# savelovme/adaptive-mcmc

Hardware: AMD Instinct MI355X
Metric: chain-steps/sec (whole node) + ESS/sec, 64-dim Gaussian (higher is better)
Workload: dtype f32; 1 GPU; ARWMH.sample, d=64 correlated Gaussian, 65536 chains, per-chain adaptation (BASELINE.json configs[1]); chains_per_gpu=65536, dim=64, parallelism=1 GPU

## Files before the change

adaptive-mcmc_amd/csrc/amh_step64.hip:

```cpp
#include "amh_asss.h"
#include "amh_device.h"
#include "amh_s64_sched.h"
#include "amh_step_stage.h"

namespace amh {

#ifdef AMH_STAMPS
constexpr int kS64StampWaves = 1 << 16;
constexpr int kS64StampSlots = 16;
constexpr int kS64SubPhases = 6;
__device__ unsigned long long g_s64_stamps[kS64StampWaves * kS64StampSlots];
hipError_t diag_s64_stamps_copy(void* host, size_t bytes) {
  return hipMemcpyFromSymbol(host, HIP_SYMBOL(g_s64_stamps), bytes, 0, hipMemcpyDeviceToHost);
}
#define AMH_S64_PHASE_INIT                                  \
  unsigned long long st_ph[4] = {0, 0, 0, 0}, st_pt = 0; \
  S64Sub st_sub = {{0, 0, 0, 0, 0, 0}, 0};
#define AMH_S64_PHASE_MARK st_pt = __builtin_amdgcn_s_memrealtime();
#define AMH_S64_PHASE(k)                                             \
  {                                                                  \
    const unsigned long long t_ = __builtin_amdgcn_s_memrealtime();  \
    st_ph[k] += t_ - st_pt;                                          \
    st_pt = t_;                                                      \
  }
struct S64Sub {
  unsigned long long ph[kS64SubPhases], pt;
};
#define AMH_S64_SUB_PARAM , S64Sub& st_sub
#define AMH_S64_SUB_ARG , st_sub
#define AMH_S64_SUB_MARK st_sub.pt = __builtin_amdgcn_s_memrealtime();
#define AMH_S64_SUB(k)                                               \
  {                                                                  \
    const unsigned long long t_ = __builtin_amdgcn_s_memrealtime();  \
    st_sub.ph[k] += t_ - st_sub.pt;                                  \
    st_sub.pt = t_;                                                  \
  }
#else
#define AMH_S64_PHASE_INIT
#define AMH_S64_PHASE_MARK
#define AMH_S64_PHASE(k)
#define AMH_S64_SUB_PARAM
#define AMH_S64_SUB_ARG
#define AMH_S64_SUB_MARK
#define AMH_S64_SUB(k)
#endif

constexpr int kS64Waves = 16;
constexpr int kS64LoadAuxHot = 2, kS64LoadAuxCold = 2;
constexpr int kS64StoreAuxHot = 2, kS64StoreAuxMid = 0, kS64StoreAuxTail = 0;
constexpr int kS64TagShift = 60;
constexpr int64_t kS64IdxMask = ((int64_t)1 << kS64TagShift) - 1;
__device__ __forceinline__ int s64_cls(int64_t t) { return (int)(t >> kS64TagShift); }
template <class F>
__device__ __forceinline__ void s64_load_policy(int cls, F&& f) {
  using std::integral_constant;
  if constexpr (kS64LoadAuxHot == kS64LoadAuxCold) {
    f(integral_constant<int, kS64LoadAuxCold>{});
  } else {
    if (cls & (int)kS64Hot) f(integral_constant<int, kS64LoadAuxHot>{});
    else f(integral_constant<int, kS64LoadAuxCold>{});
  }
}
template <class F>
__device__ __forceinline__ void s64_store_policy(int cls, F&& f) {
  using std::integral_constant;
  if constexpr (kS64StoreAuxHot == kS64StoreAuxMid && kS64StoreAuxTail == kS64StoreAuxMid) {
    f(integral_constant<int, kS64StoreAuxMid>{});
  } else {
    if (cls & (int)kS64Hot) f(integral_constant<int, kS64StoreAuxHot>{});
    else if (cls & (int)kS64Tail) f(integral_constant<int, kS64StoreAuxTail>{});
    else f(integral_constant<int, kS64StoreAuxMid>{});
  }
}
constexpr int kS64EB = 8;
constexpr int kS64PB = 8;
constexpr int kS64PG = 16;
static_assert(kS64EB == 8 && kS64PB == 8, "the batch readers (lds_ld4x2w / lds_ld4x4w) read two quarter-vectors per stream");
static_assert(kS64PG == 16, "s64_gauss_pot_sg waits for four quarter-rows; s64_lanes takes 8 or 16");
typedef uint32_t uint32x4_t_ __attribute__((ext_vector_type(4)));
constexpr int kS64P = 2080;
constexpr int kS64Z = 2080, kS64M = 2144, kS64S = 2208, kS64X = 2216;
constexpr int kS64WB = kS64X + 64;
constexpr int kS64Model = 64 * 68;
static_assert(kS64Z == 2080 && kS64S == kS64M + 64, "layout of prefetch_item<64>");
template <int WPB = kS64Waves>
constexpr size_t s64_lds_bytes() { return ((size_t)kS64Model + (size_t)WPB * kS64WB + 32) * sizeof(float); }

constexpr int s64_col(int j) { return j * 64 - j * (j - 1) / 2; }

constexpr int kS64Pieces = 9;
constexpr int s64_piece_end(int m) { return m < kS64Pieces - 1 ? 256 * (m + 1) : kS64P; }
constexpr int s64_piece_group(int m) {
  for (int g = 0; g < 16; ++g)
    if (s64_col(4 * g + 4) >= s64_piece_end(m)) return g;
  return -1;
}
constexpr int s64_piece_after(int g) {
  for (int m = 0; m < kS64Pieces; ++m)
    if (s64_piece_group(m) == g) return m;
  return -1;
}
constexpr bool s64_pieces_ok() {
  int n = 0;
  for (int g = 0; g < 16; ++g) n += s64_piece_after(g) >= 0;
  for (int m = 0; m + 1 < kS64Pieces; ++m)
    if (s64_piece_group(m) < 0 || s64_piece_group(m) >= s64_piece_group(m + 1)) return false;
  return n == kS64Pieces;
}
static_assert(256 * (kS64Pieces - 1) <= kS64P && kS64P - 256 * (kS64Pieces - 1) <= 64, "eight 1-KB pieces and a one-DMA tail");
static_assert(s64_col(64) == kS64P && s64_pieces_ok(), "every piece is finished by its own swap group, in order");
static_assert(s64_piece_group(0) == 1 && s64_piece_group(4) == 6 && s64_piece_group(7) == 14 &&
                  s64_piece_group(kS64Pieces - 1) == 15,
              "the table of DESIGN.md 3.1");

#define AMH_SWG_RD(k) "ds_read_b32 %[t" #k "], %[la] offset:%[o" #k "]\n\t"
#define AMH_SWG_RD_HEAD "ds_read_b128 %[dl], %[zm] offset:%[od]\n\tds_read_b128 %[in], %[zm] offset:%[oi]\n\t"
#define AMH_SWG_RD_PIECE "ds_read_b128 %[pv], %[lp] offset:%[op]\n\t"
#define AMH_SWG_RD_TAIL "s_waitcnt lgkmcnt(0)"
template <int G, int MP>
__device__ __forceinline__ void s64_group_read(f32x4& dl4, f32x4& in4, f32x4& pv, float (&t)[4], uint32_t zm_a,
                                               uint32_t la16, uint32_t la) {
  constexpr int j = 4 * G;
  static_assert(G < 15 || MP >= 0, "the last group reads the piece that group 14 finished");
  static_assert(s64_col(j) >= j && s64_col(j + 3) - (j + 3) + 63 < kS64P, "unmasked column reads stay inside the factor");
#define AMH_SWG_RD_OPS3                                                                          \
  [zm] "v"(zm_a), [la] "v"(la), [od] "n"(16 * G), [oi] "n"(256 + 16 * G),                       \
      [o0] "n"((s64_col(j) - j) * 4), [o1] "n"((s64_col(j + 1) - (j + 1)) * 4),                 \
      [o2] "n"((s64_col(j + 2) - (j + 2)) * 4)
  if constexpr (G == 15) {
    asm volatile(AMH_SWG_RD_HEAD AMH_SWG_RD_PIECE AMH_SWG_RD(0) AMH_SWG_RD(1) AMH_SWG_RD(2) AMH_SWG_RD_TAIL
                 : [dl] "=&v"(dl4), [in] "=&v"(in4), [pv] "=&v"(pv), [t0] "=&v"(t[0]), [t1] "=&v"(t[1]),
                   [t2] "=&v"(t[2])
                 : AMH_SWG_RD_OPS3, [lp] "v"(la16), [op] "n"(1024 * MP));
  } else if constexpr (MP >= 0) {
    asm volatile(AMH_SWG_RD_HEAD AMH_SWG_RD_PIECE AMH_SWG_RD(0) AMH_SWG_RD(1) AMH_SWG_RD(2) AMH_SWG_RD(3)
                     AMH_SWG_RD_TAIL
                 : [dl] "=&v"(dl4), [in] "=&v"(in4), [pv] "=&v"(pv), [t0] "=&v"(t[0]), [t1] "=&v"(t[1]),
                   [t2] "=&v"(t[2]), [t3] "=&v"(t[3])
                 : AMH_SWG_RD_OPS3, [o3] "n"((s64_col(j + 3) - (j + 3)) * 4), [lp] "v"(la16), [op] "n"(1024 * MP));
  } else {
    asm volatile(AMH_SWG_RD_HEAD AMH_SWG_RD(0) AMH_SWG_RD(1) AMH_SWG_RD(2) AMH_SWG_RD(3) AMH_SWG_RD_TAIL
                 : [dl] "=&v"(dl4), [in] "=&v"(in4), [t0] "=&v"(t[0]), [t1] "=&v"(t[1]), [t2] "=&v"(t[2]),
                   [t3] "=&v"(t[3])
                 : AMH_SWG_RD_OPS3, [o3] "n"((s64_col(j + 3) - (j + 3)) * 4));
  }
#undef AMH_SWG_RD_OPS3
}
#define AMH_SWG_LP                                                                      \
  "v_mul_f32 %[d0], %[u0], %[d0]\n\tv_mul_f32 %[d1], %[u1], %[d1]\n\t"                  \
  "v_mul_f32 %[d2], %[u2], %[d2]\n\tv_mul_f32 %[d3], %[u3], %[d3]\n\t"
#define AMH_SWG_WR(k) "ds_write_b32 %[la], %[d" #k "] offset:%[o" #k "]\n\t"
#define AMH_SWG_NRM(k) "v_mul_f32 %[u" #k "], %[t" #k "], %[i" #k "]\n\t"
#define AMH_SWG_SH(k) "s_lshl_b64 exec, -1, %[m" #k "]\n\t"
#define AMH_SWG_OFFS                                                                                          \
  [o0] "n"((s64_col(j) - j) * 4), [o1] "n"((s64_col(j + 1) - (j + 1)) * 4),                                   \
      [o2] "n"((s64_col(j + 2) - (j + 2)) * 4), [o3] "n"((s64_col(j + 3) - (j + 3)) * 4), [m0] "n"(j),        \
      [m1] "n"(j + 1), [m2] "n"(j + 2), [m3] "n"(j + 3)
template <int G>
__device__ __forceinline__ void s64_group_write(const float (&U)[64], uint32_t la, const f32x4& dl4) {
  constexpr int j = 4 * G;
  float d0 = dl4[0], d1 = dl4[1], d2 = dl4[2], d3 = dl4[3];
  asm volatile(AMH_SWG_LP AMH_SWG_SH(0) AMH_SWG_WR(0) AMH_SWG_SH(1) AMH_SWG_WR(1) AMH_SWG_SH(2) AMH_SWG_WR(2)
                   AMH_SWG_SH(3) AMH_SWG_WR(3) "s_mov_b64 exec, -1"
               : [d0] "+v"(d0), [d1] "+v"(d1), [d2] "+v"(d2), [d3] "+v"(d3)
               : [la] "v"(la), [u0] "v"(U[j]), [u1] "v"(U[j + 1]), [u2] "v"(U[j + 2]), [u3] "v"(U[j + 3]), AMH_SWG_OFFS
               : "memory");
}
template <int G>
__device__ __forceinline__ void s64_group_norm(float (&U)[64], const f32x4& in4, const float (&t)[4]) {
  constexpr int j = 4 * G;
  if constexpr (G < 15) {
    asm volatile(AMH_SWG_SH(1) AMH_SWG_NRM(0) AMH_SWG_SH(2) AMH_SWG_NRM(1) AMH_SWG_SH(3) AMH_SWG_NRM(2) AMH_SWG_SH(4)
                     AMH_SWG_NRM(3) "s_mov_b64 exec, -1"
                 : [u0] "+v"(U[j]), [u1] "+v"(U[j + 1]), [u2] "+v"(U[j + 2]), [u3] "+v"(U[j + 3])
                 : [t0] "v"(t[0]), [t1] "v"(t[1]), [t2] "v"(t[2]), [t3] "v"(t[3]), [i0] "v"(in4[0]), [i1] "v"(in4[1]),
                   [i2] "v"(in4[2]), [i3] "v"(in4[3]), [m1] "n"(j + 1), [m2] "n"(j + 2), [m3] "n"(j + 3),
                   [m4] "n"(j + 4));
  } else {
    asm volatile(AMH_SWG_SH(1) AMH_SWG_NRM(0) AMH_SWG_SH(2) AMH_SWG_NRM(1) AMH_SWG_SH(3) AMH_SWG_NRM(2)
                 "s_mov_b64 exec, -1"
                 : [u0] "+v"(U[j]), [u1] "+v"(U[j + 1]), [u2] "+v"(U[j + 2])
                 : [t0] "v"(t[0]), [t1] "v"(t[1]), [t2] "v"(t[2]), [i0] "v"(in4[0]), [i1] "v"(in4[1]),
                   [i2] "v"(in4[2]), [m1] "n"(j + 1), [m2] "n"(j + 2), [m3] "n"(j + 3));
  }
}
template <int O0, int O1>
__device__ __forceinline__ void lds_ld4x2w(f32x4& a, f32x4& b, uint32_t addr) {
  asm volatile("ds_read_b128 %0, %2 offset:%3\n\tds_read_b128 %1, %2 offset:%4\n\ts_waitcnt lgkmcnt(0)"
               : "=&v"(a), "=&v"(b)
               : "v"(addr), "n"(O0), "n"(O1));
}
template <int O0, int O1, int O2, int O3>
__device__ __forceinline__ void lds_ld4x4w(f32x4& a, f32x4& b, f32x4& c, f32x4& d, uint32_t addr0, uint32_t addr1) {
  asm volatile("ds_read_b128 %0, %4 offset:%6\n\tds_read_b128 %1, %4 offset:%7\n\t"
               "ds_read_b128 %2, %5 offset:%8\n\tds_read_b128 %3, %5 offset:%9\n\ts_waitcnt lgkmcnt(0)"
               : "=&v"(a), "=&v"(b), "=&v"(c), "=&v"(d)
               : "v"(addr0), "v"(addr1), "n"(O0), "n"(O1), "n"(O2), "n"(O3));
}

#define AMH_SW1_COL(k)                                                          \
  "s_lshl_b64 exec, -1, %[s" #k "]\n\tv_readlane_b32 %[t], %[w], %[l" #k "]\n\t" \
  "s_nop 1\n\tv_fma_f32 %[w], -%[t], %[u" #k "], %[w]\n\ts_nop 0\n\t"
template <int J0>
__device__ __forceinline__ void s64_sweep1x8(float& w, const float (&U)[64]) {
  uint64_t sv;
  uint32_t t;
  if constexpr (J0 + 7 <= 62) {
    asm volatile("s_mov_b64 %[sv], exec\n\t" AMH_SW1_COL(0) AMH_SW1_COL(1) AMH_SW1_COL(2) AMH_SW1_COL(3)
                 AMH_SW1_COL(4) AMH_SW1_COL(5) AMH_SW1_COL(6) AMH_SW1_COL(7) "s_mov_b64 exec, %[sv]"
                 : [w] "+v"(w), [t] "=&s"(t), [sv] "=&s"(sv)
                 : [u0] "v"(U[J0]), [u1] "v"(U[J0 + 1]), [u2] "v"(U[J0 + 2]), [u3] "v"(U[J0 + 3]),
                   [u4] "v"(U[J0 + 4]), [u5] "v"(U[J0 + 5]), [u6] "v"(U[J0 + 6]), [u7] "v"(U[J0 + 7]),
                   [s0] "n"(J0 + 1), [s1] "n"(J0 + 2), [s2] "n"(J0 + 3), [s3] "n"(J0 + 4), [s4] "n"(J0 + 5),
                   [s5] "n"(J0 + 6), [s6] "n"(J0 + 7), [s7] "n"(J0 + 8), [l0] "n"(J0), [l1] "n"(J0 + 1),
                   [l2] "n"(J0 + 2), [l3] "n"(J0 + 3), [l4] "n"(J0 + 4), [l5] "n"(J0 + 5), [l6] "n"(J0 + 6),
                   [l7] "n"(J0 + 7));
  } else {
    static_assert(J0 == 56, "sweep 1 covers columns 0 .. 62");
    asm volatile("s_mov_b64 %[sv], exec\n\t" AMH_SW1_COL(0) AMH_SW1_COL(1) AMH_SW1_COL(2) AMH_SW1_COL(3)
                 AMH_SW1_COL(4) AMH_SW1_COL(5) AMH_SW1_COL(6) "s_mov_b64 exec, %[sv]"
                 : [w] "+v"(w), [t] "=&s"(t), [sv] "=&s"(sv)
                 : [u0] "v"(U[J0]), [u1] "v"(U[J0 + 1]), [u2] "v"(U[J0 + 2]), [u3] "v"(U[J0 + 3]),
                   [u4] "v"(U[J0 + 4]), [u5] "v"(U[J0 + 5]), [u6] "v"(U[J0 + 6]), [s0] "n"(J0 + 1),
                   [s1] "n"(J0 + 2), [s2] "n"(J0 + 3), [s3] "n"(J0 + 4), [s4] "n"(J0 + 5), [s5] "n"(J0 + 6),
                   [s6] "n"(J0 + 7), [l0] "n"(J0), [l1] "n"(J0 + 1), [l2] "n"(J0 + 2), [l3] "n"(J0 + 3),
                   [l4] "n"(J0 + 4), [l5] "n"(J0 + 5), [l6] "n"(J0 + 6));
  }
}
#undef AMH_SW1_COL
__device__ __forceinline__ void s64_sweep1_all(float& w, const float (&U)[64]) {
  static_for<8>([&](auto B) {
    s64_sweep1x8<8 * B>(w, U);
    __builtin_amdgcn_sched_barrier(0);
  });
}

template <int Q>
__device__ __forceinline__ void s64_wr4_quarter(uint32_t a, float v0, float v1, float v2, float v3) {
  uint64_t sv;
  asm volatile("s_mov_b64 %0, exec\n\ts_bfm_b64 exec, 16, %6\n\tds_write_b32 %1, %2\n\t"
               "ds_write_b32 %1, %3 offset:64\n\tds_write_b32 %1, %4 offset:128\n\t"
               "ds_write_b32 %1, %5 offset:192\n\ts_mov_b64 exec, %0"
               : "=&s"(sv) : "v"(a), "v"(v0), "v"(v1), "v"(v2), "v"(v3), "n"(16 * Q) : "memory");
}
__device__ __forceinline__ void s64_wr(uint32_t a, float v) {
  asm volatile("ds_write_b32 %0, %1" : : "v"(a), "v"(v) : "memory");
}
template <int OFF>
__device__ __forceinline__ void s64_wr_off(uint32_t a, float v) {
  asm volatile("ds_write_b32 %0, %1 offset:%2" : : "v"(a), "v"(v), "n"(OFF) : "memory");
}
__device__ __forceinline__ void s64_wait() { asm volatile("s_waitcnt lgkmcnt(0)" ::: "memory"); }
template <class T>
__device__ __forceinline__ void s64_tie(T& a) { asm volatile("s_waitcnt lgkmcnt(0)" : "+v"(a)); }
template <class T>
__device__ __forceinline__ void s64_tie(T& a, T& b) { asm volatile("s_waitcnt lgkmcnt(0)" : "+v"(a), "+v"(b)); }

template <int J>
__device__ __forceinline__ float s64_keep_at(float old, float v) {
  float out;
  unsigned long long m;
  asm("s_lshl_b64 %1, 1, %4\n\tv_cndmask_b32_e64 %0, %2, %3, %1" : "=v"(out), "=&s"(m) : "v"(old), "v"(v), "n"(J));
  return out;
}

template <int J0, int N>
__device__ __forceinline__ void s64_lanes(float v, float (&s)[N]) {
  static_assert(N == 8 || N == 16, "batches of 8 or 16 lanes");
  static_for<N>([&](auto K) { s[(int)K] = __int_as_float(__builtin_amdgcn_readlane(__float_as_int(v), J0 + K)); });
  if constexpr (N == 8) {
    asm volatile("" : "+s"(s[0]), "+s"(s[1]), "+s"(s[2]), "+s"(s[3]), "+s"(s[4]), "+s"(s[5]), "+s"(s[6]), "+s"(s[7]));
  } else {
    asm volatile("" : "+s"(s[0]), "+s"(s[1]), "+s"(s[2]), "+s"(s[3]), "+s"(s[4]), "+s"(s[5]), "+s"(s[6]), "+s"(s[7]),
                 "+s"(s[8]), "+s"(s[9]), "+s"(s[10]), "+s"(s[11]), "+s"(s[12]), "+s"(s[13]), "+s"(s[14]), "+s"(s[15]));
  }
}

__device__ __forceinline__ float s64_matvec_sg(const float (&U)[64], float h) {
  float a4[4] = {0.0f, 0.0f, 0.0f, 0.0f};
  static_for<64 / kS64EB>([&](auto B) {
    constexpr int b = B;
    float e[kS64EB];
    s64_lanes<kS64EB * b>(h, e);
    static_for<kS64EB>([&](auto K) {
      constexpr int j = kS64EB * b + K;
      a4[j & 3] = fmaf(U[j], e[(int)K], a4[j & 3]);
    });
    __builtin_amdgcn_sched_barrier(0);
  });
  return (a4[0] + a4[1]) + (a4[2] + a4[3]);
}

__device__ __forceinline__ float s64_gauss_pot_sg(float diff, uint32_t prow, float c0) {
  f32x2v y01 = {0.0f, 0.0f}, y23 = {0.0f, 0.0f};
  static_for<64 / kS64PG>([&](auto B) {
    constexpr int b = B;
    constexpr int NQ = kS64PG / 4;
    f32x4 pv[NQ];
    static_for<NQ>([&](auto Q) { pv[(int)Q] = lds_ld4<16 * (NQ * b + Q)>(prow); });
    float dv[kS64PG];
    s64_lanes<kS64PG * b>(diff, dv);
    asm volatile("s_waitcnt lgkmcnt(0)" : "+v"(pv[0]), "+v"(pv[1]), "+v"(pv[2]), "+v"(pv[3]));
    static_for<2 * NQ>([&](auto K2) {
      const f32x4 q = pv[(int)K2 / 2];
      const f32x2v pp = (K2 % 2 == 0) ? f32x2v{q[0], q[1]} : f32x2v{q[2], q[3]};
      const f32x2v bp = {dv[2 * (int)K2], dv[2 * (int)K2 + 1]};
      if constexpr (K2 % 2 == 0) {
        y01 = __builtin_elementwise_fma(pp, bp, y01);
      } else {
        y23 = __builtin_elementwise_fma(pp, bp, y23);
      }
    });
    __builtin_amdgcn_sched_barrier(0);
  });
  const float y = (y01[0] + y01[1]) + (y23[0] + y23[1]);
  const float S = Grp<64>::sum(diff * y);
  return (0.5f * S) + c0;
}

template <bool WAIT = false>
__device__ __forceinline__ float s64_matvec(const float (&U)[64], float h, uint32_t x_a, uint32_t r) {
  s64_wr(x_a + r * 4u, h);
  float a4[4] = {0.0f, 0.0f, 0.0f, 0.0f};
  static_for<64 / kS64EB>([&](auto B) {
    constexpr int b = B;
    f32x4 e[kS64EB / 4];
    lds_ld4x2w<16 * (2 * b), 16 * (2 * b + 1)>(e[0], e[1], x_a);
    static_for<kS64EB>([&](auto K) {
      constexpr int j = kS64EB * b + K;
      a4[j & 3] = fmaf(U[j], e[(int)K / 4][(int)K % 4], a4[j & 3]);
    });
    __builtin_amdgcn_sched_barrier(0);
  });
  if constexpr (WAIT) s64_wait();
  return (a4[0] + a4[1]) + (a4[2] + a4[3]);
}

__device__ __forceinline__ float s64_gauss_pot(float diff, uint32_t x_a, uint32_t prow, uint32_t r, float c0) {
  s64_wr(x_a + r * 4u, diff);
  f32x2v y01 = {0.0f, 0.0f}, y23 = {0.0f, 0.0f};
  static_for<64 / kS64PB>([&](auto B) {
    constexpr int b = B;
    constexpr int NQ = kS64PB / 4;
    f32x4 pv[NQ], dv[NQ];
    lds_ld4x4w<16 * (2 * b), 16 * (2 * b + 1), 16 * (2 * b), 16 * (2 * b + 1)>(pv[0], pv[1], dv[0], dv[1], prow, x_a);
    static_for<2 * NQ>([&](auto K2) {
      const f32x4 q = pv[(int)K2 / 2];
      const f32x4 dq = dv[(int)K2 / 2];
      const f32x2v pp = (K2 % 2 == 0) ? f32x2v{q[0], q[1]} : f32x2v{q[2], q[3]};
      const f32x2v bp = (K2 % 2 == 0) ? f32x2v{dq[0], dq[1]} : f32x2v{dq[2], dq[3]};
      if constexpr (K2 % 2 == 0) {
        y01 = __builtin_elementwise_fma(pp, bp, y01);
      } else {
        y23 = __builtin_elementwise_fma(pp, bp, y23);
      }
    });
    __builtin_amdgcn_sched_barrier(0);
  });
  const float y = (y01[0] + y01[1]) + (y23[0] + y23[1]);
  const float S = Grp<64>::sum(diff * y);
  return (0.5f * S) + c0;
}

struct S64Coef {
  bool revert;
  float c, q;
};
__device__ __forceinline__ S64Coef s64_rank_one_coef(float ws, float Dg, float one, float gamma, int r) {
  using Gp = Grp<64>;
  const float gw2 = gamma * (ws * ws);
  const float tsc = gw2 / Dg;
  const float b = 1.0f + Gp::excl_scan(tsc, r);
  const float g2 = (b * Dg) + gw2;
  const float dn = g2 / b;
  const float c = (gamma * ws) / g2;
  const float q = sqrtf(dn);
  const float dnew = fmaf(c, 0.0f, one) * q;
  return {Gp::any(amh_isnan(dnew)), c, q};
}
__device__ __forceinline__ float s64_sweep2(float (&U)[64], float delta, float ws, float c, float ac, float bc,
                                            uint32_t x_a, uint32_t xq_a) {
  float s4[4] = {0.0f, 0.0f, 0.0f, 0.0f};
  float w = delta;
  static_for<16>([&](auto G4) {
    constexpr int g = G4;
    if constexpr (g % 4 == 0) s64_wr4_quarter<g / 4>(xq_a, ws, c, ac, bc);
    constexpr int gq = g % 4;
    f32x4 cw, cc, ca, cb;
    lds_ld4x4w<16 * gq, 64 + 16 * gq, 128 + 16 * gq, 192 + 16 * gq>(cw, cc, ca, cb, x_a, x_a);
    static_for<4>([&](auto Q) {
      constexpr int j = 4 * g + Q;
      const float uo = U[j];
      w = fmaf(-cw[(int)Q], uo, w);
      const float un = fmaf(cc[(int)Q], w, uo);
      const float tt = fmaf(uo, ca[(int)Q], cb[(int)Q] * w);
      s4[j & 3] = fmaf(tt, tt, s4[j & 3]);
      U[j] = un;
    });
    column_fence<g, 2>();
  });
  const float sacc = (s4[0] + s4[1]) + (s4[2] + s4[3]);
  return Grp<64>::sum(sacc);
}

__device__ __forceinline__ void asss_transition64(const StepParams& p, float (&U)[64], float& dl, float& x, float& mu,
                                                  float& pe, float& asc, bool& updated, int32_t it, uint32_t k0,
                                                  uint32_t k1, int r, const GaussianM<64>::Ctx& mctx, uint32_t x_a,
                                                  uint32_t xq_a, uint32_t prow) {
  using Gp = Grp<64>;
  constexpr int d = 64;
  const float sd = sqrtf((float)d);
  const float epsd = p.eps * sd;
  const float fd = (float)d;
  const uint32_t ur = (uint32_t)r;
  const amh_u32x4 o = amh_philox4x32_10((uint32_t)r, (uint32_t)it, 0u, AMH_TAG_ASSS, k0, k1);
  float v = amh_normal_from_bits(o.v[0]);
  float vd = amh_normal_from_bits(Gp::template bcast_u<0>(o.v[1]));
  const float ut = amh_unif01_from_bits(Gp::template bcast_u<0>(o.v[2]));
  const float th0 = 6.28318548f * amh_unif01_from_bits(Gp::template bcast_u<0>(o.v[3]));

  const float e = dl * sd;
  const float Dr = (dl + p.eps) * sd;
  const float invD = 1.0f / Dr;
  float b = x - mu;
  float y = 0.0f;
  static_for<d>([&](auto J) {
    constexpr int j = J;
    const float yl = b * invD;
    y = s64_keep_at<j>(y, yl);
    const float gj = Gp::template bcast<j>(yl * e);
    b = fmaf(-U[j], gj, b);
    column_fence<j>();
  });

  const float ns = Gp::sum(y * y);
  const float den = ns + 1.0f;
  const float zr = (2.0f * y) / den;
  const float zd = (ns - 1.0f) / den;

  const float dot = Gp::sum(v * zr) + (vd * zd);
  v = fmaf(-dot, zr, v);
  vd = fmaf(-dot, zd, vd);
  const float nv = sqrtf(Gp::sum(v * v) + (vd * vd));
  const bool degen = !(nv > 0.0f);
  v = degen ? 0.0f : v / nv;
  vd = degen ? 0.0f : vd / nv;

  const float Sz = s64_matvec<true>(U, e * zr, x_a, ur) + epsd * zr;
  const float Sv = s64_matvec<true>(U, e * v, x_a, ur) + epsd * v;

  auto x_at = [&](float c, float s, float& om) -> float {
    const float zdt = (zd * c) + (vd * s);
    om = 1.0f - zdt;
    return (((Sz * c) + (Sv * s)) / om) + mu;
  };
  auto pot = [&](float xv) -> float {
    const float u = s64_gauss_pot(xv - mctx.mr, x_a, prow, ur, mctx.c0);
    s64_wait();
    return u;
  };

  float om0;
  const float x0 = x_at(1.0f, 0.0f, om0);
  const float U0 = pot(x0);
  const float tpe = (U0 + fd * amh_logf(om0)) - amh_logf(ut);

  float th = th0, thmin = th0 - 6.28318548f, thmax = th0;
  int32_t iter = 0;
  float xt, ux;
  bool cont;
  {
    float s, c, om;
    amh_sincosf(th, &s, &c);
    xt = x_at(c, s, om);
    ux = pot(xt);
    float pt = ux + fd * amh_logf(om);
    if (amh_isnan(pt)) pt = INFINITY;
    cont = !degen && ((pt > tpe) || (om < p.eps));
  }
  while (cont) {
    const float thmin_n = (th < 0.0f) ? th : thmin;
    const float thmax_n = (th >= 0.0f) ? th : thmax;
    const amh_u32x4 ok = amh_philox4x32_10((uint32_t)iter, (uint32_t)it, 1u, AMH_TAG_ASSS, k0, k1);
    const float th_n = thmin_n + (thmax_n - thmin_n) * amh_unif01_from_bits(ok.v[0]);
    float s, c, om;
    amh_sincosf(th_n, &s, &c);
    const float xn = x_at(c, s, om);
    const float un = pot(xn);
    float pt = un + fd * amh_logf(om);
    if (amh_isnan(pt)) pt = INFINITY;
    thmin = thmin_n;
    thmax = thmax_n;
    th = th_n;
    xt = xn;
    ux = un;
    iter += 1;
    cont = (iter < kAsssMaxIter) && ((pt > tpe) || (om < p.eps));
  }
  const bool capped = degen || iter >= kAsssMaxIter;
  const float xnew = capped ? x0 : xt;
  float pen = capped ? U0 : ux;
  if (amh_isnan(pen)) pen = INFINITY;

  const int32_t itr = it + 1;
  const int32_t n = (it < p.W) ? itr : itr - p.W;
  const float gamma = lookup_gamma<64>(p, n);
  const float delta = xnew - mu;
  const float mun = mu + gamma * delta;
  const float dmu = mun - mu;
  const float locd = sqrtf(Gp::sum(dmu * dmu));

  const float sq = sqrtf(1.0f - gamma);
  const float ajj = sq * dl;
  const float Dg = ajj * ajj;
  const float one = (amh_isfinite(ajj) && ajj != 0.0f) ? 1.0f : __int_as_float(0x7FC00000);
  float ws = delta;
  s64_sweep1_all(ws, U);
  const S64Coef k = s64_rank_one_coef(ws, Dg, one, gamma, r);
  float sdiff = 0.0f;
  if (!k.revert) {
    sdiff = sqrtf(s64_sweep2(U, delta, ws, k.c, k.q - dl, k.c * k.q, x_a, xq_a));
    dl = k.q;
    updated = true;
  }
  asc = locd + sdiff;
  x = xnew;
  pe = pen;
  mu = mun;
}

__device__ __forceinline__ void arwmh_transition64(const StepParams& p, float (&U)[64], float& dl, float& z, float& mu,
                                                   float& pe, float& macc, float& lam, float& asc, bool& updated,
                                                   int32_t& nacc, int32_t it, uint32_t k0, uint32_t k1, int r,
                                                   const GaussianM<64>::Ctx& mctx, uint32_t x_a, uint32_t xq_a,
                                                   uint32_t prow, bool sg AMH_S64_SUB_PARAM) {
  using Gp = Grp<64>;
  AMH_S64_SUB_MARK
  float xi, u;
  step_noise_w64(r, (uint32_t)it, k0, k1, xi, u);

  AMH_S64_SUB(0)
  const float el = amh_expf(lam);
  const float eta = dl * xi;
  const float acc = sg ? s64_matvec_sg(U, eta) : s64_matvec(U, eta, x_a, (uint32_t)r);
  const float zp = z + fmaf(el, acc, p.eps * xi);

  AMH_S64_SUB(1)
  float pep = sg ? s64_gauss_pot_sg(zp - mctx.mr, prow, mctx.c0)
                 : s64_gauss_pot(zp - mctx.mr, x_a, prow, (uint32_t)r, mctx.c0);
  if (amh_isnan(pep)) pep = INFINITY;
  AMH_S64_SUB(2)

  const float ex = amh_expf(pe - pep);
  const float alpha = (ex > 1.0f) ? 1.0f : ex;
  const bool accept = u < alpha;
  const float zn = accept ? zp : z;
  const float pen = accept ? pep : pe;
  nacc += accept ? 1 : 0;

  const int32_t itr = it + 1;
  const int32_t n = (it < p.W) ? itr : itr - p.W;
  const float gamma = lookup_gamma<64>(p, n);
  const float maccn = macc + (alpha - macc) / (float)n;

  const float delta = zn - mu;
  const float mun = mu + gamma * delta;
  const float lamn = lam + gamma * (alpha - p.target);
  const float e1 = amh_expf(lamn);

  const float sq = sqrtf(1.0f - gamma);
  const float ajj = sq * dl;
  const float Dg = ajj * ajj;
  const float one = (amh_isfinite(ajj) && ajj != 0.0f) ? 1.0f : __int_as_float(0x7FC00000);

  AMH_S64_SUB(3)
  float ws = delta;
  s64_sweep1_all(ws, U);

  const S64Coef k = s64_rank_one_coef(ws, Dg, one, gamma, r);
  AMH_S64_SUB(4)
  if (!k.revert) {
    const float ac = (k.q * e1) - (dl * el);
    const float bc = (k.c * k.q) * e1;
    asc = sqrtf(s64_sweep2(U, delta, ws, k.c, ac, bc, x_a, xq_a));
    dl = k.q;
    updated = true;
  } else {
    const float ac = (dl * e1) - (dl * el);
    float s4[4] = {0.0f, 0.0f, 0.0f, 0.0f};
    static_for<64>([&](auto J) {
      const float tt = U[J] * Gp::template bcast<J>(ac);
      s4[J & 3] = fmaf(tt, tt, s4[J & 3]);
      column_fence<J>();
    });
    const float sacc = (s4[0] + s4[1]) + (s4[2] + s4[3]);
    asc = sqrtf(Gp::sum(sacc));
  }

  AMH_S64_SUB(5)
  z = zn;
  pe = pen;
  macc = maccn;
  mu = mun;
  lam = lamn;
}

template <int WPB, bool kASSS = false>
__global__ __launch_bounds__(WPB * 64) void arwmh_step64_kernel(StepParams p) {
  const StepParams& p_outer = p;
  constexpr int D = 64;
  constexpr uint32_t P = kS64P;
  static_assert(WPB >= 1 && (WPB * 64) % 64 == 0, "d = 64 step kernel: every wave of the block is full");
  using Gp = Grp<64>;
  using M = GaussianM<64>;
  extern __shared__ float lds[];
  M::stage(lds, p.model, D);
  float* tick = lds + kS64Model + WPB * kS64WB;
  const int64_t blk_lo = p.C * (int64_t)blockIdx.x / gridDim.x;
  const int64_t blk_hi = p.C * ((int64_t)blockIdx.x + 1) / gridDim.x;
  const uint32_t tk_step = p.descending ? ~0u : 1u;
  if (threadIdx.x == 0) {
    const S64Sched sch = s64_sched((uint32_t)(blk_hi - blk_lo), p.descending, p.chained);
    tick[0] = __uint_as_float(sch.first);
    tick[4] = __uint_as_float(sch.hot_lo);
    tick[5] = __uint_as_float(sch.hot_n);
    tick[6] = __uint_as_float(sch.tail_lo);
    tick[7] = __uint_as_float(sch.tail_n);
  }
  __syncthreads();
  const auto mctx = M::prepare(p.model, D, lane_id());
#ifdef AMH_STAMPS
  const unsigned long long st_start = __builtin_amdgcn_s_memrealtime();
  int st_items = 0;
#endif
  AMH_S64_PHASE_INIT

  const int64_t C = p.C;
  const int wave_in_block = __builtin_amdgcn_readfirstlane((int)(threadIdx.x / 64));
  float* wb = lds + kS64Model + wave_in_block * kS64WB;
  const uint32_t wb_a = lds_addr(wb);
  const uint32_t x_a = wb_a + kS64X * 4;
  const uint32_t zm_a = wb_a + kS64Z * 4;
  const uint32_t xq_a = x_a + (uint32_t)(lane_id() & 15) * 4u;
  const uint32_t prow = lds_addr(lds) + (uint32_t)lane_id() * (uint32_t)(M::ld(D) * 4);

  float U[D];
  static_for<D>([&](auto J) { U[J] = set_one_at<64, J>(0.0f, lane_id()); });
  float dl = 0.0f, z = 0.0f, mu = 0.0f, pe = 0.0f, macc = 0.0f, lam = 0.0f, asc = 0.0f;
  int32_t it = 0, nacc = 0, acc0 = 0;
  uint32_t k0 = 0, k1 = 0;
  int64_t prev = -1;
  bool prev_upd = false;

  const int64_t kEnd = blk_hi;
  const uint32_t tk_addr = lds_addr(tick);
  auto ticket = [&]() -> int64_t {
    uint32_t v = 0;
    if (lane_id() == 0) {
      uint32x4_t_ b;
      asm volatile("ds_add_rtn_u32 %0, %2, %3\n\tds_read_b128 %1, %2 offset:16\n\ts_waitcnt lgkmcnt(0)"
                   : "=&v"(v), "=&v"(b) : "v"(tk_addr), "v"(tk_step) : "memory");
      const uint32_t cls = s64_class(v, b[0], b[1], b[2], b[3]);
      v = (v < 0x3FFFFFFFu ? v : 0x3FFFFFFFu) | (cls << 30);
    }
    const uint32_t w = (uint32_t)__builtin_amdgcn_readfirstlane((int)v);
    return (blk_lo + (int64_t)(w & 0x3FFFFFFFu)) | ((int64_t)(w >> 30) << kS64TagShift);
  };
  auto ix = [](int64_t t) -> int64_t { return t & kS64IdxMask; };
  auto prefetch = [&](int64_t t, int ln) {
    s64_load_policy(s64_cls(t), [&](auto AUX) { prefetch_item<64, false, decltype(AUX)::value>(p, ix(t), D, wb, ln); });
  };

  auto store_small = [&](int64_t c, int r) {
    const StepParams& p = reload_kernarg(p_outer);
    p.out.z[c * D + r] = z;
    p.out.loc[c * D + r] = mu;
    if (r == 0) {
      p.out.i[c] = it;
      p.out.potential_energy[c] = pe;
      if constexpr (!kASSS) {
        p.out.mean_accept_prob[c] = macc;
        p.out.log_step_size[c] = lam;
      }
      p.out.as_change[c] = asc;
      p.out.rng_key[2 * c] = k0;
      p.out.rng_key[2 * c + 1] = k1;
      if (!kASSS && p.accept_count != nullptr) p.accept_count[c] = acc0 + nacc;
    }
  };
  auto copy_verbatim = [&](int64_t c, int r) {
    const uint32_t vrow = (uint32_t)r * 4u;
    const Buf Lout(uniform_ptr(p.out.scale + c * P), P * 4u);
    const Buf Lin(uniform_ptr(p.in.scale + c * P), P * 4u);
    static_for<4>([&](auto B) {
      static_for<16>([&](auto K) {
        constexpr int j = 16 * B + K;
        U[j] = Lin.ld(off_from<64, j>(vrow, kOOB, r), (uint32_t)(s64_col(j) - j) * 4u);
      });
      static_for<16>([&](auto K) {
        constexpr int j = 16 * B + K;
        Lout.st(U[j], off_from<64, j>(vrow, kOOB, r), (uint32_t)(s64_col(j) - j) * 4u);
      });
      __builtin_amdgcn_sched_barrier(0);
    });
    __builtin_amdgcn_s_waitcnt(0);
    static_for<D>([&](auto J) { U[J] = set_one_at<64, J>(0.0f, r); });
  };
  auto flush_aux = [&](int64_t c, auto AUX) {
    const Buf Lout(uniform_ptr(p.out.scale + c * P), P * 4u);
    const uint32_t la = wb_a + (uint32_t)lane_id() * 16u;
    static_for<3>([&](auto G) {
      f32x4 v[3];
      static_for<3>([&](auto Q) { v[(int)Q] = lds_ld4<1024 * (3 * G + Q)>(la); });
      asm volatile("s_waitcnt lgkmcnt(0)" : "+v"(v[0]), "+v"(v[1]), "+v"(v[2]));
      static_for<3>([&](auto Q) {
        __builtin_amdgcn_raw_buffer_store_b128(__builtin_bit_cast(uint32x4_t_, v[(int)Q]), Lout.rs,
                                               (int)(1024u * (3 * G + Q) + 16u * (uint32_t)lane_id()), 0,
                                               (int)AUX);
      });
    });
  };
  auto flush_factor = [&](int64_t t) {
    s64_store_policy(s64_cls(t), [&](auto AUX) { flush_aux(ix(t), AUX); });
  };

  int64_t item = ticket();
  int64_t nxt = ix(item) < kEnd ? ticket() : kEnd;
  if (ix(item) < kEnd) prefetch(item, lane_id());
  for (; ix(item) < kEnd;) {
    int lane = lane_id();
    asm volatile("" : "+v"(lane));
    const int r = lane;
    const uint32_t la = wb_a + (uint32_t)r * 4u;

    AMH_S64_PHASE_MARK
    __builtin_amdgcn_s_waitcnt(0x0F70);
    AMH_S64_PHASE(0)
    __builtin_amdgcn_s_setprio(3);
    if (prev >= 0) store_small(ix(prev), r);
    const bool wr = prev >= 0 && prev_upd;
    if (prev >= 0 && !prev_upd) copy_verbatim(ix(prev), r);

    float lnew = lds_ld1<0>(wb_a + (uint32_t)s64_col(r) * 4u);
    s64_tie(lnew);
    const float inv = (amh_isfinite(lnew) && lnew != 0.0f) ? 1.0f / lnew : 0.0f;
    {
      float zz = lds_ld1<kS64Z * 4>(la), mm = lds_ld1<kS64M * 4>(la);
      const uint32_t sa = wb_a + kS64S * 4;
      float s0 = lds_ld1<0>(sa), s1 = lds_ld1<4>(sa), s2 = lds_ld1<8>(sa), s3 = lds_ld1<12>(sa);
      float s4v = lds_ld1<16>(sa), s5 = lds_ld1<20>(sa), s6 = lds_ld1<24>(sa);
      asm volatile("s_waitcnt lgkmcnt(0)" : "+v"(zz), "+v"(mm), "+v"(s0), "+v"(s1), "+v"(s2), "+v"(s3), "+v"(s4v),
                   "+v"(s5), "+v"(s6));
      z = zz;
      mu = mm;
      it = __builtin_amdgcn_readfirstlane(__float_as_int(s0));
      pe = s1;
      macc = s2;
      lam = s3;
      asc = s4v;
      k0 = (uint32_t)__builtin_amdgcn_readfirstlane(__float_as_int(s5));
      k1 = (uint32_t)__builtin_amdgcn_readfirstlane(__float_as_int(s6));
      s64_wr(zm_a + (uint32_t)r * 4u, dl);
      s64_wr_off<256>(zm_a + (uint32_t)r * 4u, inv);
      dl = lnew;
      acc0 = (!kASSS && p.accept_count != nullptr && r == 0) ? p.accept_count[ix(item)] : 0;
    }

    const bool have_nxt = ix(nxt) < kEnd;
    const Buf Lnx(uniform_ptr(p.in.scale + ix(nxt) * P), P * 4u);
    auto piece_in = [&](auto M) {
      constexpr int m = M;
      if (!have_nxt) return;
      uint32_t base = wb_a;
      asm volatile("" : "+s"(base));
      lds_void* dst = (lds_void*)(uintptr_t)(base + 1024u * m);
      s64_load_policy(s64_cls(nxt), [&](auto AUX) {
        if constexpr (m < kS64Pieces - 1) {
          __builtin_amdgcn_raw_ptr_buffer_load_lds(Lnx.rs, dst, 16, (int)(16u * lane), 1024 * m, 0, (int)AUX);
        } else {
          if (256 * m + lane < kS64P)
            __builtin_amdgcn_raw_ptr_buffer_load_lds(Lnx.rs, dst, 4, (int)(4u * lane), 1024 * m, 0, (int)AUX);
        }
      });
    };
    const Buf Lout(uniform_ptr(p.out.scale + ix(wr ? prev : item) * P), P * 4u);
    const int cls = s64_cls(prev);
    const uint32_t la16 = wb_a + (uint32_t)lane * 16u;
    auto piece_out = [&](auto M, const f32x4& v) {
      constexpr int m = M;
      s64_store_policy(cls, [&](auto AUX) {
        __builtin_amdgcn_raw_buffer_store_b128(__builtin_bit_cast(uint32x4_t_, v), Lout.rs,
                                               (int)(16u * (uint32_t)lane), 1024 * m, (int)AUX);
      });
    };
    static_for<16>([&](auto G4) {
      constexpr int g = G4;
      constexpr int mp = g > 0 ? s64_piece_after(g - 1) : -1;
      f32x4 dl4, in4, pv;
      float t[4];
      s64_group_read<g, mp>(dl4, in4, pv, t, zm_a, la16, la);
      if (wr) {
        if constexpr (mp >= 0) {
          piece_out(std::integral_constant<int, mp>{}, pv);
          piece_in(std::integral_constant<int, mp>{});
          if constexpr (mp == 0) {
            AMH_S64_PHASE(1)
          }
        }
        s64_group_write<g>(U, la, dl4);
      }
      s64_group_norm<g>(U, in4, t);
    });
    if (wr) {
      constexpr int mp = s64_piece_after(15);
      static_assert(mp == kS64Pieces - 1, "the last group finishes the tail");
      f32x4 pv = lds_ld4<1024 * mp>(la16);
      s64_tie(pv);
      piece_out(std::integral_constant<int, mp>{}, pv);
      piece_in(std::integral_constant<int, mp>{});
    } else {
      AMH_S64_PHASE(1)
      s64_wait();
      static_for<kS64Pieces>([&](auto M) { piece_in(M); });
    }

    s64_wait();
    int64_t nxt2 = kEnd;
    if (have_nxt) {
      prefetch_item_small<64, false>(p, ix(nxt), D, wb, lane);
      nxt2 = ticket();
    }
    __builtin_amdgcn_s_setprio(0);
    AMH_S64_PHASE(2)

    nacc = 0;
    bool updated = false;
    const bool sg = p.n_steps == 1;
    for (int32_t t = 0; t < p.n_steps; ++t) {
      if constexpr (kASSS) {
        asss_transition64(p, U, dl, z, mu, pe, asc, updated, it, k0, k1, r, mctx, x_a, xq_a, prow);
      } else {
        arwmh_transition64(p, U, dl, z, mu, pe, macc, lam, asc, updated, nacc, it, k0, k1, r, mctx, x_a, xq_a, prow,
                           sg AMH_S64_SUB_ARG);
      }
      it += 1;
      if (p.col_z != nullptr || p.col_pe != nullptr) {
        if ((t + 1) % p.thinning == 0) {
          const int64_t kk = t / p.thinning;
          if (p.col_z != nullptr) p.col_z[(kk * C + ix(item)) * D + r] = z;
          if (p.col_pe != nullptr && r == 0) p.col_pe[kk * C + ix(item)] = pe;
        }
      }
    }
    prev = item;
    prev_upd = Gp::any(updated);
    item = nxt;
    nxt = nxt2;
    AMH_S64_PHASE(3)
#ifdef AMH_STAMPS
    ++st_items;
#endif
  }
  if (prev >= 0) {
    int lane = lane_id();
    asm volatile("" : "+v"(lane));
    const uint32_t la = wb_a + (uint32_t)lane * 4u;
    store_small(ix(prev), lane);
    if (prev_upd) {
      s64_wr(x_a + (uint32_t)lane * 4u, dl);
      static_for<16>([&](auto G4) {
        constexpr int g = G4;
        f32x4 dl4 = lds_ld4<16 * g>(x_a);
        s64_tie(dl4);
        s64_group_write<g>(U, la, dl4);
      });
      flush_factor(prev);
    } else {
      copy_verbatim(ix(prev), lane);
    }
  }
  __builtin_amdgcn_s_waitcnt(0);
#ifdef AMH_STAMPS
  {
    const unsigned long long st_end = __builtin_amdgcn_s_memrealtime();
    const int64_t w = (int64_t)blockIdx.x * WPB + wave_in_block;
    if (w < kS64StampWaves && lane_id() == 0) {
      unsigned long long* row = g_s64_stamps + w * kS64StampSlots;
      row[0] = st_start;
      row[1] = st_end;
      row[2] = (unsigned long long)st_items;
      row[3] = (unsigned long long)blockIdx.x;
      for (int k_ = 0; k_ < 4; ++k_) row[4 + k_] = st_ph[k_];
      for (int k_ = 0; k_ < kS64SubPhases; ++k_) row[8 + k_] = st_sub.ph[k_];
    }
  }
#endif
}

template <int WPB, bool kASSS = false>
hipError_t launch_step64(const StepParams& p, hipStream_t s) {
  constexpr size_t shm = s64_lds_bytes<WPB>();
  static_assert(shm <= 163840, "d = 64 step kernel: LDS budget");
  auto kern = arwmh_step64_kernel<WPB, kASSS>;
  int per_cu = 0;
  hipError_t e = hipOccupancyMaxActiveBlocksPerMultiprocessor(&per_cu, kern, WPB * 64, shm);
  if (e != hipSuccess) return e;
  const int cus = cu_count();
  if (per_cu < 1) per_cu = 1;
  const int64_t need = (p.C + WPB - 1) / WPB;
  int64_t blocks = (int64_t)cus * per_cu;
  if (blocks > need) blocks = need;
  if (blocks < 1) blocks = 1;
  hipLaunchKernelGGL(kern, dim3((unsigned)blocks), dim3(WPB * 64), shm, s, p);
  return hipGetLastError();
}

hipError_t run_step64(const StepParams& p, hipStream_t s) { return launch_step64<kS64Waves>(p, s); }
constexpr int kAsss64Waves = 16;
hipError_t run_asss_step64(const StepParams& p, hipStream_t s) {
  return launch_step64<kAsss64Waves, true>(p, s);
}

}
```

Measured before the change: 322.3 million chain-steps/s.

## Broadcast sweep2 coefficients via DPP row_newbcast and template the single-step path

The rank-one update sweep now writes each quarter's coefficients to LDS and reads back one value per lane, then broadcasts across columns with DPP row_newbcast in inline asm instead of loading four 4-wide vectors per group. This is meant to cut LDS read traffic and vector register pressure in the hot sweep. It also turns the runtime single-step flag into a template parameter, so the launcher picks a dedicated kernel instantiation when n_steps is 1. The cost is more hand-written asm with DPP hazards (s_nop) and an extra kernel variant.

Result: faster. 327.7 million chain-steps/s, median of 6 (+1.7%).

```diff
diff --git a/adaptive-mcmc_amd/csrc/amh_step64.hip b/adaptive-mcmc_amd/csrc/amh_step64.hip
--- a/adaptive-mcmc_amd/csrc/amh_step64.hip
+++ b/adaptive-mcmc_amd/csrc/amh_step64.hip
@@ -235,14 +235,6 @@
   });
 }
 
-template <int Q>
-__device__ __forceinline__ void s64_wr4_quarter(uint32_t a, float v0, float v1, float v2, float v3) {
-  uint64_t sv;
-  asm volatile("s_mov_b64 %0, exec\n\ts_bfm_b64 exec, 16, %6\n\tds_write_b32 %1, %2\n\t"
-               "ds_write_b32 %1, %3 offset:64\n\tds_write_b32 %1, %4 offset:128\n\t"
-               "ds_write_b32 %1, %5 offset:192\n\ts_mov_b64 exec, %0"
-               : "=&s"(sv) : "v"(a), "v"(v0), "v"(v1), "v"(v2), "v"(v3), "n"(16 * Q) : "memory");
-}
 __device__ __forceinline__ void s64_wr(uint32_t a, float v) {
   asm volatile("ds_write_b32 %0, %1" : : "v"(a), "v"(v) : "memory");
 }
@@ -378,25 +370,47 @@
   const float dnew = fmaf(c, 0.0f, one) * q;
   return {Gp::any(amh_isnan(dnew)), c, q};
 }
+template <int Q>
+__device__ __forceinline__ void s64_rows_quarter(uint32_t a, float v0, float v1, float v2, float v3, float& o0,
+                                                 float& o1, float& o2, float& o3) {
+  uint64_t sv;
+  asm volatile("s_mov_b64 %[sv], exec\n\ts_bfm_b64 exec, 16, %[q]\n\tds_write_b32 %[a], %[v0]\n\t"
+               "ds_write_b32 %[a], %[v1] offset:64\n\tds_write_b32 %[a], %[v2] offset:128\n\t"
+               "ds_write_b32 %[a], %[v3] offset:192\n\ts_mov_b64 exec, %[sv]\n\t"
+               "ds_read_b32 %[o0], %[a]\n\tds_read_b32 %[o1], %[a] offset:64\n\t"
+               "ds_read_b32 %[o2], %[a] offset:128\n\tds_read_b32 %[o3], %[a] offset:192\n\t"
+               "s_waitcnt lgkmcnt(0)"
+               : [sv] "=&s"(sv), [o0] "=&v"(o0), [o1] "=&v"(o1), [o2] "=&v"(o2), [o3] "=&v"(o3)
+               : [a] "v"(a), [v0] "v"(v0), [v1] "v"(v1), [v2] "v"(v2), [v3] "v"(v3), [q] "n"(16 * Q)
+               : "memory");
+}
+#define AMH_SW2_COL(k)                                                                              \
+  "v_fmac_f32_dpp %[w], -%[cw], %[u" #k "] row_newbcast:%[l" #k "] row_mask:0xf bank_mask:0xf\n\t"  \
+  "v_mul_f32_dpp %[t" #k "], %[cb], %[w] row_newbcast:%[l" #k "] row_mask:0xf bank_mask:0xf\n\t"    \
+  "v_fmac_f32_dpp %[t" #k "], %[ca], %[u" #k "] row_newbcast:%[l" #k "] row_mask:0xf bank_mask:0xf\n\t" \
+  "v_fmac_f32_dpp %[u" #k "], %[cc], %[w] row_newbcast:%[l" #k "] row_mask:0xf bank_mask:0xf\n\t"
+template <int G>
+__device__ __forceinline__ void s64_sweep2_group(float (&U)[64], float& w, float (&t)[4], float cw, float cc, float ca,
+                                                 float cb) {
+  constexpr int j = 4 * G, l = j % 16;
+  asm("s_nop 1\n\t" AMH_SW2_COL(0) AMH_SW2_COL(1) AMH_SW2_COL(2) AMH_SW2_COL(3)
+      : [w] "+v"(w), [u0] "+v"(U[j]), [u1] "+v"(U[j + 1]), [u2] "+v"(U[j + 2]), [u3] "+v"(U[j + 3]), [t0] "=&v"(t[0]),
+        [t1] "=&v"(t[1]), [t2] "=&v"(t[2]), [t3] "=&v"(t[3])
+      : [cw] "v"(cw), [cc] "v"(cc), [ca] "v"(ca), [cb] "v"(cb), [l0] "n"(l), [l1] "n"(l + 1), [l2] "n"(l + 2),
+        [l3] "n"(l + 3));
+}
+#undef AMH_SW2_COL
 __device__ __forceinline__ float s64_sweep2(float (&U)[64], float delta, float ws, float c, float ac, float bc,
-                                            uint32_t x_a, uint32_t xq_a) {
+                                            uint32_t xq_a) {
   float s4[4] = {0.0f, 0.0f, 0.0f, 0.0f};
   float w = delta;
+  float cw = 0.0f, cc = 0.0f, ca = 0.0f, cb = 0.0f;
   static_for<16>([&](auto G4) {
     constexpr int g = G4;
-    if constexpr (g % 4 == 0) s64_wr4_quarter<g / 4>(xq_a, ws, c, ac, bc);
-    constexpr int gq = g % 4;
-    f32x4 cw, cc, ca, cb;
-    lds_ld4x4w<16 * gq, 64 + 16 * gq, 128 + 16 * gq, 192 + 16 * gq>(cw, cc, ca, cb, x_a, x_a);
-    static_for<4>([&](auto Q) {
-      constexpr int j = 4 * g + Q;
-      const float uo = U[j];
-      w = fmaf(-cw[(int)Q], uo, w);
-      const float un = fmaf(cc[(int)Q], w, uo);
-      const float tt = fmaf(uo, ca[(int)Q], cb[(int)Q] * w);
-      s4[j & 3] = fmaf(tt, tt, s4[j & 3]);
-      U[j] = un;
-    });
+    if constexpr (g % 4 == 0) s64_rows_quarter<g / 4>(xq_a, ws, c, ac, bc, cw, cc, ca, cb);
+    float t[4];
+    s64_sweep2_group<g>(U, w, t, cw, cc, ca, cb);
+    static_for<4>([&](auto Q) { s4[(int)Q] = fmaf(t[(int)Q], t[(int)Q], s4[(int)Q]); });
     column_fence<g, 2>();
   });
   const float sacc = (s4[0] + s4[1]) + (s4[2] + s4[3]);
@@ -519,7 +533,7 @@
   const S64Coef k = s64_rank_one_coef(ws, Dg, one, gamma, r);
   float sdiff = 0.0f;
   if (!k.revert) {
-    sdiff = sqrtf(s64_sweep2(U, delta, ws, k.c, k.q - dl, k.c * k.q, x_a, xq_a));
+    sdiff = sqrtf(s64_sweep2(U, delta, ws, k.c, k.q - dl, k.c * k.q, xq_a));
     dl = k.q;
     updated = true;
   }
@@ -529,11 +543,12 @@
   mu = mun;
 }
 
+template <bool sg>
 __device__ __forceinline__ void arwmh_transition64(const StepParams& p, float (&U)[64], float& dl, float& z, float& mu,
                                                    float& pe, float& macc, float& lam, float& asc, bool& updated,
                                                    int32_t& nacc, int32_t it, uint32_t k0, uint32_t k1, int r,
                                                    const GaussianM<64>::Ctx& mctx, uint32_t x_a, uint32_t xq_a,
-                                                   uint32_t prow, bool sg AMH_S64_SUB_PARAM) {
+                                                   uint32_t prow AMH_S64_SUB_PARAM) {
   using Gp = Grp<64>;
   AMH_S64_SUB_MARK
   float xi, u;
@@ -582,7 +597,7 @@
   if (!k.revert) {
     const float ac = (k.q * e1) - (dl * el);
     const float bc = (k.c * k.q) * e1;
-    asc = sqrtf(s64_sweep2(U, delta, ws, k.c, ac, bc, x_a, xq_a));
+    asc = sqrtf(s64_sweep2(U, delta, ws, k.c, ac, bc, xq_a));
     dl = k.q;
     updated = true;
   } else {
@@ -605,8 +620,9 @@
   lam = lamn;
 }
 
-template <int WPB, bool kASSS = false>
+template <int WPB, bool kASSS = false, bool kSG = false>
 __global__ __launch_bounds__(WPB * 64) void arwmh_step64_kernel(StepParams p) {
+  static_assert(!(kASSS && kSG), "the scalar-register forms are ARWMH's");
   const StepParams& p_outer = p;
   constexpr int D = 64;
   constexpr uint32_t P = kS64P;
@@ -835,13 +851,12 @@
 
     nacc = 0;
     bool updated = false;
-    const bool sg = p.n_steps == 1;
     for (int32_t t = 0; t < p.n_steps; ++t) {
       if constexpr (kASSS) {
         asss_transition64(p, U, dl, z, mu, pe, asc, updated, it, k0, k1, r, mctx, x_a, xq_a, prow);
       } else {
-        arwmh_transition64(p, U, dl, z, mu, pe, macc, lam, asc, updated, nacc, it, k0, k1, r, mctx, x_a, xq_a, prow,
-                           sg AMH_S64_SUB_ARG);
+        arwmh_transition64<kSG>(p, U, dl, z, mu, pe, macc, lam, asc, updated, nacc, it, k0, k1, r, mctx, x_a, xq_a,
+                                prow AMH_S64_SUB_ARG);
       }
       it += 1;
       if (p.col_z != nullptr || p.col_pe != nullptr) {
@@ -897,11 +912,11 @@
 #endif
 }
 
-template <int WPB, bool kASSS = false>
+template <int WPB, bool kASSS = false, bool kSG = false>
 hipError_t launch_step64(const StepParams& p, hipStream_t s) {
   constexpr size_t shm = s64_lds_bytes<WPB>();
   static_assert(shm <= 163840, "d = 64 step kernel: LDS budget");
-  auto kern = arwmh_step64_kernel<WPB, kASSS>;
+  auto kern = arwmh_step64_kernel<WPB, kASSS, kSG>;
   int per_cu = 0;
   hipError_t e = hipOccupancyMaxActiveBlocksPerMultiprocessor(&per_cu, kern, WPB * 64, shm);
   if (e != hipSuccess) return e;
@@ -915,7 +930,9 @@
   return hipGetLastError();
 }
 
-hipError_t run_step64(const StepParams& p, hipStream_t s) { return launch_step64<kS64Waves>(p, s); }
+hipError_t run_step64(const StepParams& p, hipStream_t s) {
+  return p.n_steps == 1 ? launch_step64<kS64Waves, false, true>(p, s) : launch_step64<kS64Waves>(p, s);
+}
 constexpr int kAsss64Waves = 16;
 hipError_t run_asss_step64(const StepParams& p, hipStream_t s) {
   return launch_step64<kAsss64Waves, true>(p, s);
```
